# ChalmersPhotonicsLab/QAMpy

Hardware: AMD Instinct MI355X
Metric: equalised MSym/s (2-pol, 2 SPS) (higher is better)
Workload: dtype f32

## Files before the change

qampy_amd/csrc/api.hip:

```cpp
#include "common.h"
#include <stdlib.h>
#include <atomic>
#include <mutex>
#include <vector>
#include <unordered_map>
#include <string.h>

namespace qh {

thread_local hipStream_t g_stream = nullptr;
static thread_local hipStream_t g_streams[4] = {nullptr, nullptr, nullptr, nullptr};
int g_device = -1;
static thread_local std::string g_err;
static std::mutex g_mu;

void set_error(const std::string &s) { g_err = s; }

int hip_fail(hipError_t e, const char *what, const char *file, int line)
{
    g_err = std::string(hipGetErrorString(e)) + " in " + what + " (" + file + ":" + std::to_string(line) + ")";
    (void)hipGetLastError();
    return QH_ERR_HIP;
}

// ... 53 lines not shown
            const int reserved = reserved_cus();
            const int ncu = prop.multiProcessorCount;
            if (reserved > 0 && reserved < ncu) {
                std::vector<uint32_t> mask((ncu + 31) / 32, 0u);
                for (int c = reserved; c < ncu; c++) mask[c / 32] |= 1u << (c % 32);
                if (hipExtStreamCreateWithCUMask(&g_streams[i], (uint32_t)mask.size(), mask.data()) == hipSuccess) continue;
                (void)hipGetLastError();
                g_streams[i] = nullptr;
            }
        }
        QH_HIP(hipStreamCreateWithPriority(&g_streams[i], hipStreamNonBlocking, i == 2 ? prio_least : prio_greatest));
    }
    g_stream = g_streams[0];
    g_device = device;
    return QH_OK;
}

hipStream_t side_stream() { return g_stream == g_streams[0] ? g_streams[1] : g_streams[0]; }
hipStream_t helper_stream() { return g_streams[3]; }

int ensure_init()
{
    if (g_stream) return QH_OK;
    return init_device(g_device >= 0 ? g_device : 0);
}

thread_local void *g_scratch[SCRATCH_SLOTS] = {nullptr};
thread_local size_t g_scratch_n[SCRATCH_SLOTS] = {0};
thread_local unsigned g_scratch_epoch = 0;
static std::atomic<int> g_form[FORM_COUNT];
struct FormName { const char *key, *env; };
static const FormName FORM_NAMES[FORM_COUNT] = {
    {"trainer", "QAMPY_HIP_TRAINER"}, {"pit_form", "QAMPY_HIP_PIT_FORM"}, {"seg_lanes", "QAMPY_HIP_SEG_LANES"}, {"pit_probe", "QAMPY_HIP_PIT_PROBE"},
    {"bps", "QAMPY_HIP_BPS"}, {"pit_tail", "QAMPY_HIP_PIT_TAIL"}};
static int form_parse(int k, const char *v, int *out)
{
    if (!v || !v[0]) { *out = 0; return 0; }
    switch (k) {
    case FORM_TRAINER: *out = v[0] == 'd' ? 1 : (v[0] == 'l' ? 2 : (v[0] == 'i' ? 3 : (v[0] == 'a' || v[0] == '0' ? 0 : -1))); break;
    case FORM_PIT: *out = v[0] == 's' ? 1 : (v[0] == 'b' ? 2 : (v[0] == 'a' || v[0] == '0' ? 0 : -1)); break;
    case FORM_SEG_LANES: { const int n = atoi(v); *out = (n == 8 || n == 16 || n == 0) ? n : -1; break; }
    case FORM_BPS: *out = v[0] == 't' ? 1 : (v[0] == 'l' ? 2 : (v[0] == 'a' || v[0] == '0' ? 0 : -1)); break;
    case FORM_PIT_TAIL: *out = v[0] == 's' ? 1 : (v[0] == 'a' || v[0] == '0' ? 0 : -1); break;
    default: *out = atoi(v) != 0 ? 1 : 0; break;
    }
    return *out < 0 ? -1 : 0;
}
static const int g_form_env_read = [] {
    for (int k = 0; k < FORM_COUNT; k++) {
        int v = 0;
        if (form_parse(k, getenv(FORM_NAMES[k].env), &v) == 0) g_form[k].store(v);
    }
    return 0;
}();
int form(FormKey k) { return g_form[k].load(std::memory_order_relaxed); }
const char *trainer_force()
{
    switch (form(FORM_TRAINER)) {
    case 1: return "direct";
    case 2: return "lookahead";
    case 3: return "iterative";
    default: return "";
    }
}
static constexpr int POOL_CLASSES = 48, POOL_KEEP = 8;
static constexpr size_t POOL_BYTES = (size_t)24 << 30;
static std::vector<void *> g_pool[POOL_CLASSES];
static size_t g_pool_bytes = 0;
static void pool_release();
static int pool_class(size_t bytes) { int k = 8; while (((size_t)1 << k) < bytes && k < POOL_CLASSES - 1) k++; return k; }
int pool_alloc(size_t bytes, void **p, size_t *cap)
{
    const int k = pool_class(bytes);
    *cap = (size_t)1 << k;
    {
        std::lock_guard<std::mutex> lk(g_mu);
// ... 360 lines not shown
```

qampy_amd/csrc/common.h:

```cpp
#pragma once
#include <hip/hip_runtime.h>
#include <stdint.h>
#include <string>
#include "../../include/qampy_hip.h"

namespace qh {

extern thread_local hipStream_t g_stream;
extern int g_device;
void set_error(const std::string &s);
int hip_fail(hipError_t e, const char *what, const char *file, int line);

#define QH_HIP(call)                                                        \
    do {                                                                    \
        hipError_t _e = (call);                                             \
        if (_e != hipSuccess) return qh::hip_fail(_e, #call, __FILE__, __LINE__); \
    } while (0)

#define QH_REQUIRE(cond, msg)                                   \
    do {                                                        \
        if (!(cond)) { qh::set_error(msg); return QH_ERR_ARG; } \
    } while (0)

#define QH_WAVE_FIRST() __builtin_amdgcn_s_setprio(3)

int ensure_init();
hipStream_t side_stream();
hipStream_t helper_stream();
enum FormKey { FORM_TRAINER = 0, FORM_PIT, FORM_SEG_LANES, FORM_PIT_PROBE, FORM_BPS, FORM_PIT_TAIL, FORM_COUNT };
int form(FormKey k);
const char *trainer_force();
double gram_budget_gb();
int pit_timing_mode();
int default_tier();
double default_tier_tol();
constexpr int SCRATCH_SLOTS = 27;
constexpr int SCRATCH_TWOSTAGE = 16;
constexpr int SCRATCH_FOE = 17;
constexpr int SCRATCH_IMPAIR = 18;
constexpr int SCRATCH_PMD = 19;
constexpr int SCRATCH_TXRESP = 20;
constexpr int SCRATCH_SOS = 21;
constexpr int SCRATCH_CPR = 22;
constexpr int SCRATCH_FFT = 23;
constexpr int SCRATCH_SYNC = 24;
constexpr int SCRATCH_PEAK = 25;
constexpr int SCRATCH_PILOT = 26;
int scratch(int slot, size_t bytes, void **p);
unsigned scratch_epoch();

int bps_twostage_recover_f32(const void *E, int nm, int64_t L, const void *angles, int A, int B, const void *symbols, int M, int N, int32_t *idx1,
                             int32_t *idx2, void *ph, void *Eout);
int bps_twostage_recover_f64(const void *E, int nm, int64_t L, const void *angles, int A, int B, const void *symbols, int M, int N, int32_t *idx1,
                             int32_t *idx2, void *ph, void *Eout);

template <typename R> int fft_correlate_pow2(const void *x, int rows, int64_t nx, void *yrev, int64_t ny, int64_t P, void *spec, void *cc, int64_t n);

int pool_alloc(size_t bytes, void **p, size_t *cap);
void pool_free(void *p, size_t cap);

struct DevBuf {
    void *p = nullptr;
// ... 109 lines not shown
```

qampy_amd/csrc/train_pit.h:

```cpp
#pragma once
#include <atomic>
#include <chrono>
#include <vector>
#include "train_impl.h"
#include "train_seg.h"

namespace qh {

typedef qh_pit_report PitCtrl;

constexpr double PIT_CONTRACT = 0.2;
constexpr int PIT_PROBE = 128;
constexpr int PIT_SEEDWIN = 512;
constexpr int PIT_MAXSEG = 65536;

__host__ __device__ inline int pit_symmetry(int method)
{
    switch (method) {
    case QH_M_CMA: case QH_M_SGNCMA: case QH_M_RDE: return 0;
    case QH_M_CMA2: return 2;
    default: return 4;
    }
}

// ... 1973 lines not shown
            tp.wx = wx; tp.err = err; tp.mu = mu_acq; tp.nseg = 1; tp.seg_begin = step0; tp.seg_len = pl.CH; tp.seg_iter = 0; tp.skip = &ctrl->acq_done;
            rc = launch_any<R>(tp);
        }
        if (rc) return rc;
        hipLaunchKernelGGL((pit_acq_monitor_kernel<R>), dim3(1), dim3(256), 0, g_stream, (const Cx<R> *)err, err_pitch, step0, pl.CH, nsel, modes_dev,
                           pl.plateau, ctrl, mu_acq, mu_dev, pl.anneal);
    }
    return QH_OK;
}

struct PitPrepLayout { size_t ctrl, mu_acq, modes, wx, w0, err, gram, total; int64_t err_pitch; };
template <typename R> inline PitPrepLayout pit_prep_layout(int nmodes, int ntaps, int64_t acq_steps)
{
    PitPrepLayout l;
    auto up = [](size_t x) { return (x + 255) / 256 * 256; };
    const size_t wset = (size_t)nmodes * nmodes * ntaps * sizeof(Cx<R>);
    l.err_pitch = (acq_steps + LA_B + 63) / 64 * 64;
    l.ctrl = 0; l.mu_acq = up(sizeof(PitCtrl)); l.modes = l.mu_acq + 64; l.wx = up(l.modes + 128); l.w0 = up(l.wx + wset);
    l.err = up(l.w0 + wset); l.gram = up(l.err + (size_t)nmodes * l.err_pitch * sizeof(Cx<R>));
    l.total = up(l.gram + gram_bytes<R>(l.err_pitch));
    return l;
}
template <typename R> __global__ void __launch_bounds__(256) pit_adopt_kernel(Cx<R> *wx, const Cx<R> *wx_prep, int n, const PitCtrl *p, PitCtrl *c, R *mu_acq, const R *mu_acq_prep)
{
    QH_WAVE_FIRST();
    const int i = blockIdx.x * blockDim.x + threadIdx.x;
    if (!p->diverged && i < n) wx[i] = wx_prep[i];
    if (i == 0) {
        c->acq_chunks = p->acq_chunks; c->acq_steps = p->acq_steps; c->acq_done = 1; c->diverged = p->diverged; c->mu_acq = p->mu_acq;
        for (int q = 0; q < QH_PIT_MAXCHUNK; q++) c->acq_err[q] = p->acq_err[q];
        *mu_acq = *mu_acq_prep;
    }
}
template <typename R>
int pit_prepare(const void *E, int nmodes, int64_t L, int64_t TrSyms, int os, const R *mu_dev, const void *wx0, int ntaps, const int64_t *modes, int nsel,
                const void *symbols, int64_t nsy, int method, const qh_pit_opts *opts, void *prep, size_t prep_bytes)
{
    int rc = ensure_init();
    if (rc) return rc;
    if ((rc = train_args_ok("pit prepare", method, nmodes, ntaps, os, TrSyms, 1, nsel, nsy, modes))) return rc;
    QH_REQUIRE(opts && prep, "pit prepare: options and a preparation buffer are needed");
    QH_REQUIRE(TrSyms >= 1, "pit prepare: bad sizes");
    QH_REQUIRE((TrSyms - 1) * os + ntaps <= L, "pit prepare: field shorter than TrSyms*os + ntaps");
    const qh_pit_opts &o = *opts;
    QH_REQUIRE(o.acquire != 0 && o.adaptive == 0 && o.segments > 1 && o.mu_hint > 0 && o.acq_chunk > 0 && o.head_steps == 0 && !o.exchange,
               "pit prepare: not preparable (a cold fixed-step sweep with segments, mu_hint and acq_chunk given)");
    const int ntot = nmodes * ntaps;
    const PitPlan pl = pit_plan(o, TrSyms, 0, o.segments, false, o.acq_chunk);
    const PitSeg &sg = pl.sg;
    QH_REQUIRE(sg.S >= 2, "pit prepare: not preparable (nothing to parallelise)");
    const char *not_prep = "pit prepare: not preparable (throughput-form passes, block-form acquisition, blind error function)";
    QH_REQUIRE(!(method == QH_M_SBD || method == QH_M_MDDMA || method == QH_M_DD || method == QH_M_SBD_DATA), not_prep);
    TrainerForm f;
    if ((rc = trainer_form<R>(f, FORM_PASSES, method, 0, nmodes, ntaps, os, sg.len, (int64_t)sg.S * nsel, symbols, nsy, modes, nsel))) return rc;
    QH_REQUIRE(f.seg && f.block && la_shape_ok(nmodes, ntaps, os), not_prep);
    const PitPrepLayout lay = pit_prep_layout<R>(nmodes, ntaps, pl.amax);
    QH_REQUIRE(prep_bytes >= lay.total, "pit prepare: preparation buffer too small (qh_pit_prepare_bytes)");
    char *pb = (char *)prep;
    PitCtrl *ctrl = (PitCtrl *)(pb + lay.ctrl);
    R *mu_acq = (R *)(pb + lay.mu_acq);
    int64_t *modes_dev = (int64_t *)(pb + lay.modes);
    Cx<R> *wxp = (Cx<R> *)(pb + lay.wx), *w0 = (Cx<R> *)(pb + lay.w0), *errp = (Cx<R> *)(pb + lay.err);
    const size_t wset = (size_t)nmodes * ntot, wbytes = wset * sizeof(Cx<R>);
    const int64_t npow = L < 4096 ? L : 4096;
    hipLaunchKernelGGL((pit_setup_kernel<R>), dim3(1), dim3(256), 0, g_stream, (const Cx<R> *)E, nmodes, L, npow, ntot, mu_dev, pl.gear, pl.bound, o.tol > 0 ? o.tol : 1e-3, sg, ctrl, mu_acq);
    PitInit init{};
    init.cd[0] = wxp; init.cs[0] = wx0; init.cn[0] = (unsigned)wbytes;
    init.cd[1] = w0; init.cs[1] = wx0; init.cn[1] = (unsigned)wbytes;
    init.modes_dev = modes_dev; init.nsel = nsel;
    for (int j = 0; j < 16; j++) init.modes[j] = j < nsel ? modes[j] : 0;
    hipLaunchKernelGGL(pit_init_kernel, dim3(32), dim3(256), 0, g_stream, init);
    QH_REQUIRE(pl.ngram <= lay.err_pitch, "pit prepare: acquisition range exceeds the preparation buffer");
    void *G = nullptr;
    rc = f.pair_tab ? gram_build<R>(E, nmodes, L, os, ntaps, pl.ngram, &G, 1, 0, 0, pb + lay.gram) : QH_ERR_ARG;
    if (rc) return rc;
    LaArgs<R> la = la_args<R>(E, L, nmodes, ntaps, os, modes, nsel, method, symbols, nsy, mu_acq, errp, lay.err_pitch);
    la.G = (const GramPair<R> *)G; la.gpair = 1;
    if ((rc = pit_acq_enqueue<R>(pl, &la, f.use_bi, nullptr, wxp, errp, lay.err_pitch, ctrl, mu_acq, mu_dev, modes_dev, nsel))) return rc;
    hipLaunchKernelGGL((pit_acq_finish_kernel<R>), dim3((unsigned)((wset + 255) / 256)), dim3(256), 0, g_stream, wxp, (const Cx<R> *)w0, (int)wset, ctrl);
    QH_HIP(hipGetLastError());
    return QH_OK;
}

template <typename R>
int train_pit_dev(const void *E, int nmodes, int64_t L, int64_t TrSyms, int Niter, int os, R *mu_dev, void *wx, int ntaps,
                  const int64_t *modes, int nsel, const void *symbols, int64_t nsy, int method, void *err, int zero_err,
                  const void *gram, const qh_pit_opts *opts, void *report_dev, int depth = 0)
{
    pit_last_launch() = PitLaunch{0, 0, 0, 0, 0, 0};
    int rc = ensure_init();
    if (rc) return rc;
    if ((rc = train_args_ok("train_equaliser", method, nmodes, ntaps, os, TrSyms, Niter, nsel, nsy, modes))) return rc;
    QH_REQUIRE(TrSyms == 0 || (TrSyms - 1) * os + ntaps <= L, "train_equaliser: field shorter than TrSyms*os + ntaps");
    qh_pit_opts o = opts ? *opts : pit_opts_default();
    auto exact_form = [&](PitCtrl *c, int ad, int zero, const void *g, int passes) -> int {
        int r = train_dev<R>(E, nmodes, L, TrSyms, Niter, os, mu_dev, wx, ntaps, modes, nsel, ad, symbols, nsy, method, err, zero, g);
        if (r) return r;
        const int32_t hdr[3] = {1, passes, 2};
        if (passes < 0) QH_HIP(hipMemcpyAsync(&c->converged, &hdr[2], sizeof(int32_t), hipMemcpyHostToDevice, g_stream));
        else QH_HIP(hipMemcpyAsync(&c->segments, hdr, sizeof(hdr), hipMemcpyHostToDevice, g_stream));
        QH_HIP(hipStreamSynchronize(g_stream));
        return QH_OK;
    };
    QH_REQUIRE(o.segments >= 0 && o.segments <= PIT_MAXSEG && o.max_passes >= 0 && o.max_passes <= QH_PIT_MAXPASS, "train_equaliser: bad segment / pass count");
    QH_REQUIRE(o.adaptive >= 0 && o.adaptive <= 2, "train_equaliser: adaptive must be 0, 1 or 2");
    bool adaptive = o.adaptive != 0;
    {
        bool exact_only = method == QH_M_SBD_DATA;
        if (adaptive && (o.adaptive == 2 || sizeof(R) != 4 || nsel != 1 || Niter != 1 || !seg_adaptive_supported(method))) exact_only = true;
        QH_REQUIRE(!(adaptive && o.exchange), "train_equaliser: a capture split over processes is trained with a fixed step");
        if (exact_only) {
            QH_REQUIRE(!o.exchange, "train_equaliser: a capture split over processes needs the parallel-in-time solver (blind / decision-directed method, fixed step)");
            void *cb0 = nullptr;
            if ((rc = scratch(8, sizeof(PitCtrl) + 64, &cb0))) return rc;
            PitCtrl *c0 = report_dev ? (PitCtrl *)report_dev : (PitCtrl *)cb0;
            PitSeg s1; s1.S = 1; s1.len = TrSyms; s1.extra = 0; s1.tail = 0;
            hipLaunchKernelGGL((pit_setup_kernel<R>), dim3(1), dim3(256), 0, g_stream, (const Cx<R> *)E, nmodes, L, (int64_t)(L < 4096 ? L : 4096), nmodes * ntaps, (const R *)mu_dev, 1.0, 1.0,
                               o.tol > 0 ? o.tol : 1e-3, s1, c0, (R *)((char *)cb0 + sizeof(PitCtrl)));
            return exact_form(c0, o.adaptive, zero_err, adaptive ? nullptr : gram, 0);
        }
    }
    if (adaptive) o.acquire = 0;
    const int ntot = nmodes * ntaps;
    const int npass = o.max_passes > 0 ? o.max_passes : (adaptive ? QH_PIT_MAXPASS : 16);
    const double tol = (o.tol > 0 ? o.tol : 1e-3) * (adaptive ? 1.0 / 3.0 : 1.0);
    const double safety = o.dev_safety > 0 ? o.dev_safety : PIT_DEV_SAFETY;
    const int sym = pit_symmetry(method);
    const bool seed_phase = o.phase_seed < 0 ? sym == 4 : o.phase_seed != 0;
    const bool want_corr = o.correction != 0 && pit_basis_ok(ntot, sizeof(Cx<R>));
    double beta = o.corr_beta >= 0 ? o.corr_beta : (sym == 0 ? 1.5 : 0.0);

    void *cbuf = nullptr;
    if ((rc = scratch(8, sizeof(PitCtrl) + 64, &cbuf))) return rc;
    PitCtrl *ctrl = report_dev ? (PitCtrl *)report_dev : (PitCtrl *)cbuf;
    R *mu_acq = (R *)((char *)cbuf + sizeof(PitCtrl));

    int S = o.segments;
    const float ad_relax = 1.0f, ad_damp = 0.7f;
    const int ad_newton = 1;
    const int64_t head_want = 16384;
    int64_t head = adaptive ? ((TrSyms / 4 < head_want ? TrSyms / 4 : head_want) / LA_B * LA_B) : 0;
    if (!adaptive && o.head_steps > 0) {
        QH_REQUIRE(!o.exchange, "train_equaliser: a capture split over processes takes no exact head");
        head = (int64_t)o.head_steps / LA_B * LA_B;
        if (head > TrSyms) head = TrSyms / LA_B * LA_B;
        o.acquire = 0;
    }
    int64_t seg_want = 2048;
    if (adaptive && !(method == QH_M_SBD || method == QH_M_MDDMA || method == QH_M_DD)) {
        const int64_t t = ((TrSyms - head) / 512 + LA_B - 1) / LA_B * LA_B;
        if (t > seg_want) seg_want = t;
    }
    if (S == 0 && adaptive) S = (int)((TrSyms - head) / seg_want < PIT_MAXSEG ? (TrSyms - head) / seg_want : PIT_MAXSEG);
    if (S == 0) {
        R mu_h = (R)o.mu_hint;
        if (!(o.mu_hint > 0)) {
            QH_HIP(hipMemcpyAsync(&mu_h, mu_dev, sizeof(R), hipMemcpyDeviceToHost, g_stream));
            QH_HIP(hipStreamSynchronize(g_stream));
        }
        S = pit_auto_segments(TrSyms, (double)mu_h, nsel, o.acquire);
    }
    PitPlan pl = pit_plan(o, TrSyms, head, S, adaptive, o.acquire ? o.acq_chunk : 0);
    const PitSeg &sg = pl.sg;
    if (zero_err) QH_HIP(hipMemsetAsync(err, 0, (size_t)nmodes * TrSyms * Niter * sizeof(Cx<R>), g_stream));
    const int64_t npow = L < 4096 ? L : 4096;
    hipLaunchKernelGGL((pit_setup_kernel<R>), dim3(1), dim3(256), 0, g_stream, (const Cx<R> *)E, nmodes, L, npow, ntot, (const R *)mu_dev, pl.gear, pl.bound, tol, sg, ctrl, mu_acq);
    QH_HIP(hipGetLastError());
    if (TrSyms == 0 || Niter == 0) return QH_OK;
    if (sg.S < 2) {
        const double zero = 0;
        QH_HIP(hipMemcpyAsync(&ctrl->defect[0], &zero, sizeof(double), hipMemcpyHostToDevice, g_stream));
        return exact_form(ctrl, adaptive ? 1 : 0, 0, gram, 1);
    }

    TrainerForm f;
    if ((rc = trainer_form<R>(f, FORM_PASSES, method, adaptive, nmodes, ntaps, os, sg.len, (int64_t)sg.S * nsel, symbols, nsy, modes, nsel))) return rc;
    if (adaptive && !f.seg) return exact_form(ctrl, 1, 0, nullptr, 0);
    const bool decision = method == QH_M_SBD || method == QH_M_MDDMA || method == QH_M_DD;
    const bool seg_form = f.seg, use_bi = f.use_bi, block_form = f.block, pair_tab = f.pair_tab;
    const bool split = o.exchange != nullptr;
    const int own_first = split ? o.seg_first : 0, own_count = split ? o.seg_count : sg.S;
    const bool xchg_async = split && o.exchange_on_stream != 0;
    if (split) {
        QH_REQUIRE(seg_form, "train_equaliser: a capture split over processes needs the throughput form of the passes (>= 512 chains, supported tap layout)");
        QH_REQUIRE(own_first >= 0 && own_count >= 0 && own_first + own_count <= sg.S, "train_equaliser: owned segments outside the segment grid");
        QH_REQUIRE(Niter == 1, "train_equaliser: a capture split over processes is trained in one sweep");
    }

    const size_t wset = (size_t)nmodes * ntot;
    const size_t wbytes = wset * sizeof(Cx<R>);
    void *wbuf = nullptr;
    const size_t nsj = (size_t)sg.S * nsel;
    const size_t bytes_w = ((2 * (size_t)sg.S + 2) * wbytes + 63) / 64 * 64;
    if ((rc = scratch(2, bytes_w + 10 * nsj * sizeof(double) + (size_t)nsel * sizeof(int64_t) + 320 + nsj * 16 + 4 * ((nsj + 63) / 64) * sizeof(float) + 64, &wbuf))) return rc;
    Cx<R> *X = (Cx<R> *)wbuf, *Y = X + (size_t)sg.S * wset, *w_start = Y + (size_t)sg.S * wset, *w_call = w_start + wset;
    double *z = (double *)((char *)wbuf + bytes_w), *rot = z + 2 * nsj, *dfc = rot + 2 * nsj, *pw = dfc + nsj, *gph = pw + nsj, *theta = gph + 2 * nsj;
    int64_t *modes_dev = (int64_t *)(theta + 2 * nsj);
    double *uw_phi = (double *)(modes_dev + ((nsel + 7) / 8 * 8));
    int *uw_jump = (int *)(uw_phi + (size_t)sg.S * nsel);
    float *devmax = (float *)(uw_jump + (size_t)sg.S * nsel);
    const int ndev = (int)((nsj + 63) / 64);
    unsigned *ticket = (unsigned *)(devmax + 4 * (size_t)ndev);
    PitInit init{};
    init.z[0] = ticket; init.zn[0] = sizeof(unsigned);
    R *ad_rS = nullptr, *ad_rE = nullptr;
    Cx<R> *ad_eS = nullptr, *ad_eE = nullptr, *ad_errh = nullptr;
    float *ad_M = nullptr, *ad_chg = nullptr, *ad_rP = nullptr, *ad_dP = nullptr;
    if (!adaptive && head > 0) {
        void *ab = nullptr;
        if ((rc = scratch(13, (size_t)nmodes * head * sizeof(Cx<R>) + 64, &ab))) return rc;
        ad_errh = (Cx<R> *)ab;
    }
    if (adaptive) {
        void *ab = nullptr;
        const size_t nS = ((size_t)sg.S + 15) / 16 * 16;
        if ((rc = scratch(13, nS * (2 * sizeof(R) + 2 * sizeof(Cx<R>) + 3 * sizeof(float)) + 64 + (size_t)nmodes * head * sizeof(Cx<R>), &ab))) return rc;
        ad_eS = (Cx<R> *)ab; ad_eE = ad_eS + nS; ad_errh = ad_eE + nS;
        ad_rS = (R *)(ad_errh + (size_t)nmodes * head); ad_rE = ad_rS + nS;
        ad_M = (float *)(ad_rE + nS); ad_rP = ad_M + nS; ad_dP = ad_rP + nS; ad_chg = ad_dP + nS;
    }
    init.modes_dev = modes_dev; init.nsel = nsel;
    for (int j = 0; j < 16; j++) init.modes[j] = j < nsel ? modes[j] : 0;
    const bool prepared = o.prepared != nullptr && o.acquire && !adaptive && head == 0 && Niter >= 1;
    const bool need_mu = adaptive || !(o.mu_hint > 0), need_acq = o.acquire && !(o.acq_chunk > 0) && !prepared;
    R mu_acq_h = 0;
    if (need_acq) QH_HIP(hipMemcpyAsync(&mu_acq_h, mu_acq, sizeof(R), hipMemcpyDeviceToHost, g_stream));
    R mu_host = need_mu ? (R)1 : (R)o.mu_hint;
    if (need_mu) QH_HIP(hipMemcpyAsync(&mu_host, mu_dev, sizeof(R), hipMemcpyDeviceToHost, g_stream));
    if (need_mu || need_acq) QH_HIP(hipStreamSynchronize(g_stream));
    if (!adaptive && !(mu_host != 0))
        return exact_form(ctrl, 0, 0, gram, 0);
    if (o.acquire && !(o.acq_chunk > 0)) pl.acquisition(o, TrSyms, pit_acq_chunk(mu_acq_h));

    const int64_t amax = pl.amax;
    void *G = const_cast<void *>(gram);
    if (prepared) QH_REQUIRE(seg_form && o.acq_chunk > 0, "train_equaliser: a prepared acquisition belongs to throughput-form passes with acq_chunk given (qh_pit_prepare_*_dev said so)");
    if (block_form && !G && (!seg_form || amax > 0) && !prepared) {
        const int64_t n = seg_form ? pl.ngram : TrSyms;
        rc = pair_tab ? gram_build<R>(E, nmodes, L, os, ntaps, n, &G) : gram_cur_build<R>(E, nmodes, L, os, ntaps, n, &G);
        if (rc) return rc;
    }
    const int64_t g_per_step = pair_tab ? LA_B : GRAM_TRI / 2 / LA_B;

    const int ncol = sg.S * nsel;
    const double *lam = nullptr;
    const Zf *Vb = nullptr;
    Zf *Dz[2] = {nullptr, nullptr};
    Zf *Xe = nullptr, *Ye = nullptr, *Yprev = nullptr;
    if (want_corr) {
        void *cb = nullptr;
        if ((rc = scratch(10, pit_basis_bytes(ntot) + 4 * (size_t)ntot * ncol * sizeof(Zf) + (size_t)ntot * nsel * sizeof(Zf) + 256, &cb))) return rc;
        void *basis = o.basis ? o.basis : cb;
        if (!o.basis && (rc = pit_basis<R>(E, nmodes, L, os, ntaps, TrSyms, basis))) return rc;
        lam = (const double *)basis; Vb = (const Zf *)((const char *)basis + (size_t)ntot * sizeof(double));
        Dz[0] = (Zf *)((char *)cb + (pit_basis_bytes(ntot) + 63) / 64 * 64); Dz[1] = Dz[0] + (size_t)ntot * ncol;
        Xe = Dz[1] + (size_t)ntot * ncol; Ye = Xe + (size_t)ntot * ncol; Yprev = Ye + (size_t)ntot * ncol;
    }
// ... 18 lines not shown
        model = (PitModel *)((char *)uqv + b_uq); ma.model = model; ma.ticket = (unsigned *)(model + 16);
        init.z[1] = ma.ticket; init.zn[1] = sizeof(unsigned);
        init.z[2] = ualpha; init.zn[2] = (unsigned)(b_ua + b_uq);
        ma.E = (const Cx<R> *)E; ma.wx = (const Cx<R> *)wx; ma.L = L; ma.TrSyms = TrSyms; ma.nmodes = nmodes; ma.ntaps = ntaps; ma.os = os; ma.nsel = nsel; ma.method = method;
        if (decision) { ma.symbols = (const Cx<R> *)f.dd_table; ma.nsy = 2 * f.dd_npart + 1; ma.sy_pitch = 2 * BI_DD_MAXLEV; ma.tables = 1; }
        else { ma.symbols = (const Cx<R> *)symbols; ma.nsy = nsy; ma.sy_pitch = nsy; ma.tables = (method == QH_M_RDE || method == QH_M_MRDE) ? 1 : 0; }
        for (int j = 0; j < 16; j++) ma.modes[j] = j < nsel ? modes[j] : 0;
        if (o.corr_beta < 0) beta = 0.0;
    }
    const size_t glds = ((size_t)PIT_EIGMAX * PIT_EIGMAX + (size_t)PIT_EIGMAX * PIT_GT) * sizeof(Zf);
    static std::atomic<bool> gemm_attr{false};
    if (want_corr && !gemm_attr.load(std::memory_order_acquire)) {
        QH_HIP(hipFuncSetAttribute((const void *)pit_cgemm_kernel<R, true>, hipFuncAttributeMaxDynamicSharedMemorySize, 160 * 1024 - 256));
        QH_HIP(hipFuncSetAttribute((const void *)pit_cgemm_kernel<R, false>, hipFuncAttributeMaxDynamicSharedMemorySize, 160 * 1024 - 256));
        QH_HIP(hipFuncSetAttribute((const void *)pit_basis_mfma_kernel<R, 0>, hipFuncAttributeMaxDynamicSharedMemorySize, 128 * 1024));
        QH_HIP(hipFuncSetAttribute((const void *)pit_basis_mfma_kernel<R, 1>, hipFuncAttributeMaxDynamicSharedMemorySize, 128 * 1024));
        QH_HIP(hipFuncSetAttribute((const void *)pit_tail_kernel<R>, hipFuncAttributeMaxDynamicSharedMemorySize, 128 * 1024));
        gemm_attr.store(true, std::memory_order_release);
    }

    LaArgs<R> la = la_args<R>(E, L, nmodes, ntaps, os, modes, nsel, method, symbols, nsy, mu_dev, err, TrSyms * Niter);
    la.G = (const GramPair<R> *)G; la.gpair = pair_tab ? 1 : 0; la.wx_cs = (int64_t)wset;
    la.dd_general = f.dd_general;
    f.alphabet(la);
    const TrainArgs<R> ta = train_args<R>(E, L, nmodes, ntaps, os, TrSyms, Niter, modes, nsel, method, symbols, nsy, mu_dev, err);

    PitTiming &tm = pit_timing();
    tm.npass = 0; tm.acq_ms = 0;
    bool acq_timed = false;
    PitEvents &ev = pit_events();
    QH_REQUIRE(ev.ok, "train_equaliser: no pinned memory for the pass flags");
    const bool redo_ok = o.exact_redo_off == 0;
    bool fell_back = false;
    if (redo_ok && !adaptive) { init.cd[0] = w_call; init.cs[0] = wx; init.cn[0] = (unsigned)wbytes; }
    if (o.acquire && Niter > 0) { init.cd[1] = w_start; init.cs[1] = wx; init.cn[1] = (unsigned)wbytes; }
    hipLaunchKernelGGL(pit_init_kernel, dim3(32), dim3(256), 0, g_stream, init);
    QH_HIP(hipGetLastError());
    for (int it = 0; it < Niter; it++) {
        if (it == 0 && prepared) {
            const PitPrepLayout lay = pit_prep_layout<R>(nmodes, ntaps, amax);
            const char *pb = (const char *)o.prepared;
            hipLaunchKernelGGL((pit_adopt_kernel<R>), dim3((unsigned)((wset + 255) / 256)), dim3(256), 0, g_stream, (Cx<R> *)wx, (const Cx<R> *)(pb + lay.wx), (int)wset,
                               (const PitCtrl *)(pb + lay.ctrl), ctrl, mu_acq, (const R *)(pb + lay.mu_acq));
            QH_HIP(hipGetLastError());
        } else if (it == 0 && o.acquire) {
            if (pl.nchunks > 0) { QH_HIP(hipEventRecord(ev.t0[PIT_NEV - 1], g_stream)); acq_timed = true; }
            if ((rc = pit_acq_enqueue<R>(pl, block_form ? &la : nullptr, use_bi, &ta, (Cx<R> *)wx, (Cx<R> *)err, TrSyms * Niter, ctrl, mu_acq, mu_dev,
                                         modes_dev, nsel))) return rc;
            if (pl.nchunks > 0) QH_HIP(hipEventRecord(ev.t1[PIT_NEV - 1], g_stream));
            hipLaunchKernelGGL((pit_acq_finish_kernel<R>), dim3((unsigned)((wset + 255) / 256)), dim3(256), 0, g_stream, (Cx<R> *)wx, (const Cx<R> *)w_start, (int)wset, ctrl);
            QH_HIP(hipGetLastError());
        }
        if (adaptive) {
            QH_HIP(hipMemcpyAsync(w_start, wx, wbytes, hipMemcpyDeviceToDevice, g_stream));
            QH_HIP(hipMemcpyAsync(ad_chg + 1, mu_dev, sizeof(R), hipMemcpyDeviceToDevice, g_stream));
            if ((rc = train_dev<R>(E, nmodes, L, head, 1, os, mu_dev, wx, ntaps, modes, 1, 1, symbols, nsy, method, ad_errh, 0, nullptr))) return rc;
            QH_HIP(hipMemcpyAsync((Cx<R> *)err + (size_t)modes[0] * TrSyms, ad_errh + (size_t)modes[0] * head, (size_t)head * sizeof(Cx<R>), hipMemcpyDeviceToDevice, g_stream));
            hipLaunchKernelGGL((pit_adapt_init_kernel<R>), dim3((sg.S + 255) / 256), dim3(256), 0, g_stream, (const R *)mu_dev, (const Cx<R> *)(ad_errh + (size_t)modes[0] * head + head - 1),
                               sg.S, ad_rS, ad_eS);
            QH_HIP(hipGetLastError());
        }
        if (!adaptive && head > 0) {
            if ((rc = train_dev<R>(E, nmodes, L, head, 1, os, mu_dev, wx, ntaps, modes, nsel, 0, symbols, nsy, method, ad_errh, 0, nullptr))) return rc;
            for (int j = 0; j < nsel; j++)
                QH_HIP(hipMemcpyAsync((Cx<R> *)err + (size_t)modes[j] * TrSyms * Niter + (size_t)it * TrSyms, ad_errh + (size_t)modes[j] * head, (size_t)head * sizeof(Cx<R>),
                                      hipMemcpyDeviceToDevice, g_stream));
        }
        const double *rot_use = nullptr;
        if (seed_phase) {
            int nwin = PIT_SEEDWIN;
            auto phase_lds = [&](int nw) { return ((size_t)ntot + (size_t)nmodes * os * pit_phase_pitch(ntaps, os, nw)) * sizeof(Cx<R>); };
            while (nwin > 32 && phase_lds(nwin) > 60 * 1024) nwin /= 2;
            QH_REQUIRE(phase_lds(nwin) <= 60 * 1024, "train_equaliser: phase seeding does not fit the LDS for this filter shape (pass phase_seed = 0)");
            hipLaunchKernelGGL((pit_phase_kernel<R>), dim3(sg.S, nsel), dim3(256), phase_lds(nwin), g_stream, (const Cx<R> *)E, nmodes, L, os,
                               (const Cx<R> *)wx, ntaps, sg, (const int64_t *)modes_dev, nwin, z);
            hipLaunchKernelGGL(pit_unwrap_kernel, dim3(nsel), dim3(256), 0, g_stream, (const double *)z, sg.S, nsel, rot, uw_phi, uw_jump);
            rot_use = rot;
        }
        const Cx<R> *w_exact = o.start == 1 ? nullptr : ((it == 0 && o.acquire) ? (const Cx<R> *)w_start : (const Cx<R> *)wx);
        hipLaunchKernelGGL((pit_seed_kernel<R>), dim3(sg.S), dim3(256), 0, g_stream, (const Cx<R> *)wx, nmodes, ntot, (const int64_t *)modes_dev, nsel, rot_use, X, w_exact, Y, ctrl);
        if (ssb) {
            ma.sg = sg; ma.rot = rot_use;
            static thread_local hipEvent_t ev_seed = nullptr, ev_model = nullptr;
            if (!ev_seed) { QH_HIP(hipEventCreateWithFlags(&ev_seed, hipEventDisableTiming)); QH_HIP(hipEventCreateWithFlags(&ev_model, hipEventDisableTiming)); }
            hipStream_t ss = helper_stream();
            QH_HIP(hipEventRecord(ev_seed, g_stream));
            QH_HIP(hipStreamWaitEvent(ss, ev_seed, 0));
            hipLaunchKernelGGL((pit_model_kernel<R, 0>), dim3(PIT_MODB), dim3(256), 0, ss, ma);
            hipLaunchKernelGGL((pit_model_kernel<R, 1>), dim3(PIT_MODB), dim3(256), 0, ss, ma);
            QH_HIP(hipEventRecord(ev_model, ss));
            model_event = ev_model;
        }
        QH_HIP(hipGetLastError());
        const int timing_mode = pit_timing_mode();
        auto decide_args = [&](int p, const float *dm, const float2 *ye, float2 *yprev, int ne, int ncol_e, int corr_wanted) {
            PitDecideArgs<R> d;
            d.dfc = dfc; d.pw = pw; d.nb = (int)((sg.S - 1) * nsel); d.Ylast = (const Cx<R> *)(Y + (size_t)(sg.S - 1) * wset); d.n = (int)wset; d.wx = (Cx<R> *)wx; d.c = ctrl;
            d.host_view = &ev.hview[2 * p]; d.nrow = nsel; d.devmax = dm; d.ndev = ndev; d.safety = safety; d.Ye = ye; d.Yprev = yprev; d.ne = ne; d.ncol_e = ncol_e;
            d.theta = theta; d.modes_dev = (const int64_t *)modes_dev; d.ntot_w = ntot; d.S = (int)sg.S; d.sym = sym; d.corr_wanted = corr_wanted;
            d.extra = adaptive ? (const float *)ad_chg : nullptr;
            d.Dfin = (ye && !adaptive) ? (const float2 *)Dz[1] : nullptr; d.Vfin = (const float2 *)Vb; d.lam_fin = lam;
            d.stall_from = o.correction == 0 ? QH_PIT_MAXPASS : (adaptive ? 5 : 2);
            return d;
        };
        auto timed = [&](int p) { return timing_mode == 2 || (timing_mode == 1 && p == 1); };
        int back_done_for = 0;
        auto enqueue_pass = [&](int p) -> int {
            ((volatile float *)ev.hview)[2 * p] = -1.f;
            PitFuse<R> fz;
            fz.X = X; fz.Y = Y; fz.theta = theta; fz.modes_dev = (const int64_t *)modes_dev; fz.nmodes = nmodes; fz.nsel = nsel;
            fz.damp = (adaptive && p > 1) ? ad_damp : 1.f;
            fz.x_only = tail_fused ? 1 : 0;
            if (p > 0 && tail_fused && back_done_for == p) {
// ... 264 lines not shown
```

Baseline: 1237.

## Fuse PIT setup, init and phase-seed kernels into fewer launches

Merges the single-block setup kernel and the init/copy kernel into one multi-block open kernel, and lets the open work ride as extra blocks inside a new fused phase-estimation kernel. Phase unwrapping moves into the seed kernel, which computes the cumulative quarter-turn jumps per segment, so the separate unwrap launch goes away. The phase filter now processes two selected modes per block with vectorised FMA. This is meant to cut kernel launch count and serial single-block stages on the f32 path, at the cost of redundant per-block prefix scans and more code paths gated by an env switch.

```diff
diff --git a/qampy_amd/csrc/api.hip b/qampy_amd/csrc/api.hip
--- a/qampy_amd/csrc/api.hip
+++ b/qampy_amd/csrc/api.hip
@@ -109,7 +109,7 @@
 struct FormName { const char *key, *env; };
 static const FormName FORM_NAMES[FORM_COUNT] = {
     {"trainer", "QAMPY_HIP_TRAINER"}, {"pit_form", "QAMPY_HIP_PIT_FORM"}, {"seg_lanes", "QAMPY_HIP_SEG_LANES"}, {"pit_probe", "QAMPY_HIP_PIT_PROBE"},
-    {"bps", "QAMPY_HIP_BPS"}, {"pit_tail", "QAMPY_HIP_PIT_TAIL"}};
+    {"bps", "QAMPY_HIP_BPS"}, {"pit_tail", "QAMPY_HIP_PIT_TAIL"}, {"pit_open", "QAMPY_HIP_PIT_OPEN"}};
 static int form_parse(int k, const char *v, int *out)
 {
     if (!v || !v[0]) { *out = 0; return 0; }
@@ -118,7 +118,7 @@
     case FORM_PIT: *out = v[0] == 's' ? 1 : (v[0] == 'b' ? 2 : (v[0] == 'a' || v[0] == '0' ? 0 : -1)); break;
     case FORM_SEG_LANES: { const int n = atoi(v); *out = (n == 8 || n == 16 || n == 0) ? n : -1; break; }
     case FORM_BPS: *out = v[0] == 't' ? 1 : (v[0] == 'l' ? 2 : (v[0] == 'a' || v[0] == '0' ? 0 : -1)); break;
-    case FORM_PIT_TAIL: *out = v[0] == 's' ? 1 : (v[0] == 'a' || v[0] == '0' ? 0 : -1); break;
+    case FORM_PIT_TAIL: case FORM_PIT_OPEN: *out = v[0] == 's' ? 1 : (v[0] == 'a' || v[0] == '0' ? 0 : -1); break;
     default: *out = atoi(v) != 0 ? 1 : 0; break;
     }
     return *out < 0 ? -1 : 0;
diff --git a/qampy_amd/csrc/common.h b/qampy_amd/csrc/common.h
--- a/qampy_amd/csrc/common.h
+++ b/qampy_amd/csrc/common.h
@@ -27,7 +27,7 @@
 int ensure_init();
 hipStream_t side_stream();
 hipStream_t helper_stream();
-enum FormKey { FORM_TRAINER = 0, FORM_PIT, FORM_SEG_LANES, FORM_PIT_PROBE, FORM_BPS, FORM_PIT_TAIL, FORM_COUNT };
+enum FormKey { FORM_TRAINER = 0, FORM_PIT, FORM_SEG_LANES, FORM_PIT_PROBE, FORM_BPS, FORM_PIT_TAIL, FORM_PIT_OPEN, FORM_COUNT };
 int form(FormKey k);
 const char *trainer_force();
 double gram_budget_gb();
diff --git a/qampy_amd/csrc/train_pit.h b/qampy_amd/csrc/train_pit.h
--- a/qampy_amd/csrc/train_pit.h
+++ b/qampy_amd/csrc/train_pit.h
@@ -2029,6 +2029,258 @@
         *mu_acq = *mu_acq_prep;
     }
 }
+template <typename R> struct PitOpen {
+    const Cx<R> *E; int nmodes; int64_t L, npow; int ntot; const R *mu; double gear, bound, tol; PitSeg sg; PitCtrl *c; R *mu_acq;
+    PitInit init;
+    Cx<R> *wx, *copy0, *copy1; int n;
+    const Cx<R> *wx_prep; const PitCtrl *p; const R *mu_acq_prep;
+};
+template <typename R, int NM = 2> __device__ __forceinline__ void pit_open_body(const PitOpen<R> &a, int bid, int nblk, double *red)
+{
+    const int t = threadIdx.x;
+    if (bid == 0) {
+        PitCtrl *c = a.c;
+        const PitCtrl *p = a.p;
+        double m = 0, p_mu_acq = 0;
+        R p_mu = 0;
+        int64_t p_steps = 0;
+        int p_chunks = 0, p_div = 0;
+        if (t == 0) {
+            m = (double)*a.mu;
+            if (p) { p_mu_acq = p->mu_acq; p_mu = *a.mu_acq_prep; p_steps = p->acq_steps; p_chunks = p->acq_chunks; p_div = p->diverged; }
+        }
+        const double p_err = t < QH_PIT_MAXCHUNK && p ? p->acq_err[t] : -1;
+        constexpr int NU = 16;
+        double acc = 0;
+        for (int k0 = 0; k0 < a.nmodes; k0 += NM) {
+            Cx<R> v[NM][NU];
+#pragma unroll
+            for (int mm = 0; mm < NM; mm++)
+#pragma unroll
+                for (int u = 0; u < NU; u++) {
+                    const int64_t i = t + 256 * u;
+                    const bool in = k0 + mm < a.nmodes && i < a.npow;
+                    v[mm][u] = a.E[in ? (size_t)(k0 + mm) * a.L + i : 0];
+                }
+#pragma unroll
+            for (int mm = 0; mm < NM; mm++)
+#pragma unroll
+                for (int u = 0; u < NU; u++)
+                    if (k0 + mm < a.nmodes && t + 256 * u < a.npow) acc += (double)v[mm][u].re * v[mm][u].re + (double)v[mm][u].im * v[mm][u].im;
+        }
+        if (t < QH_PIT_MAXPASS) { c->result_change[t] = -1; c->deviation[t] = -1; c->deviation_rms[t] = -1; c->deviation_taps[t] = -1; c->deviation_taps_worst[t] = -1; c->defect[t] = -1; }
+        if (t < QH_PIT_MAXCHUNK) c->acq_err[t] = p_err;
+        red[t] = acc;
+        __syncthreads();
+        for (int s = 128; s > 0; s >>= 1) {
+            if (t < s) red[t] += red[t + s];
+            __syncthreads();
+        }
+        if (t == 0) {
+            const double pw = red[0] / ((double)a.nmodes * (double)a.npow);
+            double ma = a.gear * m;
+            const double cap = a.bound / ((double)a.ntot * (pw > 1e-30 ? pw : 1e-30));
+            if (ma > cap) ma = cap;
+            if (!(ma > m)) ma = m;
+            c->segments = a.sg.S; c->seg_len = a.sg.len; c->mu = m; c->power = pw; c->tol = a.tol;
+            c->passes = 0; c->converged = 0; c->done = 0; c->corr_on = 0; c->gain = 0; c->out_power = 0;
+            c->mu_acq = p ? p_mu_acq : ma; c->acq_chunks = p_chunks; c->acq_steps = p_steps; c->acq_done = p ? 1 : 0; c->diverged = p_div;
+            *a.mu_acq = p ? p_mu : (R)ma;
+        }
+        __syncthreads();
+    }
+    if (nblk > 1 && bid == 0) return;
+    const unsigned g = (nblk > 1 ? bid - 1 : 0) * 256 + t, ng = (nblk > 1 ? nblk - 1 : 1) * 256;
+#pragma unroll
+    for (int r = 0; r < 3; r++)
+        if (a.init.z[r]) for (unsigned i = g; i < a.init.zn[r] / 4; i += ng) reinterpret_cast<uint32_t *>(a.init.z[r])[i] = 0u;
+    if ((int)g < a.init.nsel) a.init.modes_dev[g] = a.init.modes[g];
+    const bool adopt = a.p && !a.p->diverged;
+    for (unsigned e = g; e < (unsigned)a.n; e += ng) {
+        const Cx<R> v = a.wx[e];
+        if (a.copy0) a.copy0[e] = v;
+        if (a.copy1) a.copy1[e] = v;
+        if (adopt) a.wx[e] = a.wx_prep[e];
+    }
+}
+template <typename R> __global__ void __launch_bounds__(256) pit_open_kernel(PitOpen<R> a)
+{
+    QH_WAVE_FIRST();
+    __shared__ double red[256];
+    pit_open_body<R>(a, (int)blockIdx.x, (int)gridDim.x, red);
+}
+constexpr int PIT_OPEN_BLOCKS = 33;
+
+struct PitModes { int m[16]; };
+typedef float pit_f2 __attribute__((ext_vector_type(2)));
+template <typename R> __device__ __forceinline__ void pit_phase_mac(R &yr, R &yi, const Cx<R> a, const Cx<R> b)
+{
+    if constexpr (sizeof(R) == 4) {
+        pit_f2 y{yr, yi};
+        y = __builtin_elementwise_fma(pit_f2{-a.im, a.im}, pit_f2{b.im, b.re}, y);
+        y = __builtin_elementwise_fma(pit_f2{a.re, a.re}, pit_f2{b.re, b.im}, y);
+        yr = y.x; yi = y.y;
+    } else {
+        yr = fma_(a.re, b.re, fma_(-a.im, b.im, yr));
+        yi = fma_(a.re, b.im, fma_(a.im, b.re, yi));
+    }
+}
+template <typename R, int NO, int NJ>
+__device__ __forceinline__ void pit_phase_filter(const Cx<R> *xs, int pitch, const Cx<R> *__restrict__ w0, const Cx<R> *__restrict__ w1, int nmodes, int os, int ntaps, const int *at,
+                                                 R (*yr)[2], R (*yi)[2])
+{
+    constexpr int CH = 4;
+    for (int k = 0; k < nmodes; k++)
+        for (int r = 0; r < os; r++) {
+            const Cx<R> *xp = xs + ((size_t)k * os + r) * pitch;
+            const Cx<R> *wr[2] = {w0 + k * ntaps + r, w1 + k * ntaps + r};
+            const int nu = (ntaps - r + os - 1) / os;
+            int u = 0;
+            for (; u + CH <= nu; u += CH) {
+                Cx<R> b[NJ][CH], a[NO][CH];
+#pragma unroll
+                for (int jj = 0; jj < NJ; jj++)
+#pragma unroll
+                    for (int c = 0; c < CH; c++) b[jj][c] = wr[jj][(u + c) * os];
+#pragma unroll
+                for (int m = 0; m < NO; m++)
+#pragma unroll
+                    for (int c = 0; c < CH; c++) a[m][c] = xp[at[m] + u + c];
+#pragma unroll
+                for (int c = 0; c < CH; c++)
+#pragma unroll
+                    for (int jj = 0; jj < NJ; jj++)
+#pragma unroll
+                        for (int m = 0; m < NO; m++) pit_phase_mac<R>(yr[jj][m], yi[jj][m], a[m][c], b[jj][c]);
+            }
+            for (; u < nu; u++) {
+#pragma unroll
+                for (int m = 0; m < NO; m++) {
+                    const Cx<R> a = xp[at[m] + u];
+#pragma unroll
+                    for (int jj = 0; jj < NJ; jj++) pit_phase_mac<R>(yr[jj][m], yi[jj][m], a, wr[jj][u * os]);
+                }
+            }
+        }
+}
+template <typename R>
+__global__ void __launch_bounds__(256) pit_phase_open_kernel(const Cx<R> *E, int nmodes, int64_t L, int os, const Cx<R> *__restrict__ wx, int ntaps, PitSeg sg, PitModes modes,
+                                                             int nsel, int nwin, double *phi, PitOpen<R> open, int nopen)
+{
+    QH_WAVE_FIRST();
+    extern __shared__ __attribute__((aligned(16))) char pit_smem[];
+    double *rr = reinterpret_cast<double *>(pit_smem), *ri = rr + 256;
+    if ((int)blockIdx.x < nopen) { pit_open_body<R, 1>(open, (int)blockIdx.x, nopen, rr); return; }
+    static_assert(PIT_SEEDWIN == 512, "pit_phase_open_kernel: one or two outputs per thread");
+    const int ntot = nmodes * ntaps;
+    const int pitch = nwin + (ntaps + os - 1) / os + 1;
+    Cx<R> *xs = reinterpret_cast<Cx<R> *>(pit_smem);
+    const int blk = (int)blockIdx.x - nopen, s = blk % sg.S, j0 = 2 * (blk / sg.S);
+    const int nj = nsel - j0 < 2 ? 1 : 2;
+    const Cx<R> *w0 = wx + (size_t)modes.m[j0] * ntot, *w1 = wx + (size_t)modes.m[j0 + nj - 1] * ntot;
+    const int64_t st = sg.start(s);
+    int64_t n = sg.steps(s);
+    if (n > nwin) n = nwin;
+    const int ns = n > 0 ? (int)(n - 1) * os + ntaps : 0;
+    for (int k = 0; k < nmodes; k++) {
+        const Cx<R> *x = E + (size_t)k * L + st * os;
+        for (int g = threadIdx.x; g < ns; g += 256) xs[((size_t)k * os + g % os) * pitch + g / os] = x[g];
+    }
+    __syncthreads();
+    R yr[2][2] = {{0, 0}, {0, 0}}, yi[2][2] = {{0, 0}, {0, 0}};
+    int at[2];
+#pragma unroll
+    for (int m = 0; m < 2; m++) at[m] = (int)threadIdx.x + 256 * m < n ? (int)threadIdx.x + 256 * m : 0;
+    if (n > 256 && nj == 2) pit_phase_filter<R, 2, 2>(xs, pitch, w0, w1, nmodes, os, ntaps, at, yr, yi);
+    else if (n > 256) pit_phase_filter<R, 2, 1>(xs, pitch, w0, w1, nmodes, os, ntaps, at, yr, yi);
+    else if (n > 0 && nj == 2) pit_phase_filter<R, 1, 2>(xs, pitch, w0, w1, nmodes, os, ntaps, at, yr, yi);
+    else if (n > 0) pit_phase_filter<R, 1, 1>(xs, pitch, w0, w1, nmodes, os, ntaps, at, yr, yi);
+#pragma unroll
+    for (int jj = 0; jj < 2; jj++) {
+        if (jj < nj) {
+            double zr = 0, zi = 0;
+#pragma unroll
+            for (int m = 0; m < 2; m++) {
+                if ((int)threadIdx.x + 256 * m < n) {
+                    const double y2r = (double)yr[jj][m] * yr[jj][m] - (double)yi[jj][m] * yi[jj][m], y2i = 2.0 * yr[jj][m] * yi[jj][m];
+                    zr += y2r * y2r - y2i * y2i;
+                    zi += 2.0 * y2r * y2i;
+                }
+            }
+            __syncthreads();
+            rr[threadIdx.x] = zr; ri[threadIdx.x] = zi;
+            __syncthreads();
+            for (int q = 128; q > 0; q >>= 1) {
+                if (threadIdx.x < q) { rr[threadIdx.x] += rr[threadIdx.x + q]; ri[threadIdx.x] += ri[threadIdx.x + q]; }
+                __syncthreads();
+            }
+            if (threadIdx.x == 0) phi[(size_t)(j0 + jj) * sg.S + s] = (rr[0] == 0 && ri[0] == 0) ? 0.0 : (double)atan2f((float)-ri[0], (float)-rr[0]) / 4;
+        }
+    }
+}
+
+template <typename R>
+__global__ void __launch_bounds__(256) pit_seed_open_kernel(const Cx<R> *wx, int nmodes, int ntot, const int64_t *modes_dev, int nsel, const double *phi, int S, double *rot, Cx<R> *X,
+                                                            const Cx<R> *w0, Cx<R> *Y, PitCtrl *c)
+{
+    QH_WAVE_FIRST();
+    __shared__ int wsum[4];
+    __shared__ double rl[16][2];
+    const int s = blockIdx.x;
+    const int n = nmodes * ntot;
+    if (s == 0 && c) {
+        if (threadIdx.x == 0) { c->done = 0; c->converged = 0; c->passes = 0; }
+        for (int q = threadIdx.x; q < QH_PIT_MAXPASS; q += 256) {
+            c->result_change[q] = -1; c->deviation[q] = -1; c->deviation_rms[q] = -1; c->deviation_taps[q] = -1; c->deviation_taps_worst[q] = -1; c->defect[q] = -1;
+        }
+    }
+    const double q = 1.5707963267948966;
+    constexpr int NB = 8;
+    for (int j = 0; j < nsel; j++) {
+        const double *ph = phi + (size_t)j * S;
+        int jumps = 0;
+        for (int base = 1; base <= s; base += 256 * NB) {
+            double a[NB], b[NB];
+#pragma unroll
+            for (int u = 0; u < NB; u++) {
+                const int sp = base + 256 * u + (int)threadIdx.x;
+                a[u] = ph[(sp <= s ? sp : s) - 1]; b[u] = ph[sp <= s ? sp : s];
+            }
+#pragma unroll
+            for (int u = 0; u < NB; u++)
+                if (base + 256 * u + (int)threadIdx.x <= s) jumps += (int)rint((a[u] - b[u]) / q);
+        }
+        for (int o = 32; o > 0; o >>= 1) jumps += __shfl_xor(jumps, o);
+        if ((threadIdx.x & 63) == 0) wsum[threadIdx.x >> 6] = jumps;
+        __syncthreads();
+        if (threadIdx.x == 0) {
+            const double p = ph[s] + q * ((wsum[0] + wsum[1] + wsum[2] + wsum[3]) & 3);
+            float sn, cs;
+            sincosf((float)p, &sn, &cs);
+            rl[j][0] = cs; rl[j][1] = -sn;
+            rot[2 * ((size_t)s * nsel + j)] = cs;
+            rot[2 * ((size_t)s * nsel + j) + 1] = -sn;
+        }
+        __syncthreads();
+    }
+    const bool exact0 = s == 0 && w0 != nullptr;
+    for (int e = threadIdx.x; e < n; e += 256) {
+        const int row = e / ntot;
+        Cx<R> v = exact0 ? w0[e] : wx[e];
+        if (!exact0) {
+            for (int j = 0; j < nsel; j++)
+                if ((int)modes_dev[j] == row) {
+                    const double c = rl[j][0], d = rl[j][1];
+                    const double vr = (double)v.re * c - (double)v.im * d, vi = (double)v.re * d + (double)v.im * c;
+                    v = Cx<R>{(R)vr, (R)vi};
+                    break;
+                }
+        }
+        X[(size_t)s * n + e] = v;
+        Y[(size_t)s * n + e] = v;
+    }
+}
+
 template <typename R>
 int pit_prepare(const void *E, int nmodes, int64_t L, int64_t TrSyms, int os, const R *mu_dev, const void *wx0, int ntaps, const int64_t *modes, int nsel,
                 const void *symbols, int64_t nsy, int method, const qh_pit_opts *opts, void *prep, size_t prep_bytes)
@@ -2060,13 +2312,19 @@
     Cx<R> *wxp = (Cx<R> *)(pb + lay.wx), *w0 = (Cx<R> *)(pb + lay.w0), *errp = (Cx<R> *)(pb + lay.err);
     const size_t wset = (size_t)nmodes * ntot, wbytes = wset * sizeof(Cx<R>);
     const int64_t npow = L < 4096 ? L : 4096;
-    hipLaunchKernelGGL((pit_setup_kernel<R>), dim3(1), dim3(256), 0, g_stream, (const Cx<R> *)E, nmodes, L, npow, ntot, mu_dev, pl.gear, pl.bound, o.tol > 0 ? o.tol : 1e-3, sg, ctrl, mu_acq);
     PitInit init{};
-    init.cd[0] = wxp; init.cs[0] = wx0; init.cn[0] = (unsigned)wbytes;
-    init.cd[1] = w0; init.cs[1] = wx0; init.cn[1] = (unsigned)wbytes;
     init.modes_dev = modes_dev; init.nsel = nsel;
     for (int j = 0; j < 16; j++) init.modes[j] = j < nsel ? modes[j] : 0;
-    hipLaunchKernelGGL(pit_init_kernel, dim3(32), dim3(256), 0, g_stream, init);
+    if (form(FORM_PIT_OPEN) == 0 && sizeof(R) == 4) {
+        PitOpen<R> op{(const Cx<R> *)E, nmodes, L, npow, ntot, mu_dev, pl.gear, pl.bound, o.tol > 0 ? o.tol : 1e-3, sg, ctrl, mu_acq, init,
+                      (Cx<R> *)const_cast<void *>(wx0), wxp, w0, (int)wset, nullptr, nullptr, nullptr};
+        hipLaunchKernelGGL((pit_open_kernel<R>), dim3(PIT_OPEN_BLOCKS), dim3(256), 0, g_stream, op);
+    } else {
+        hipLaunchKernelGGL((pit_setup_kernel<R>), dim3(1), dim3(256), 0, g_stream, (const Cx<R> *)E, nmodes, L, npow, ntot, mu_dev, pl.gear, pl.bound, o.tol > 0 ? o.tol : 1e-3, sg, ctrl, mu_acq);
+        init.cd[0] = wxp; init.cs[0] = wx0; init.cn[0] = (unsigned)wbytes;
+        init.cd[1] = w0; init.cs[1] = wx0; init.cn[1] = (unsigned)wbytes;
+        hipLaunchKernelGGL(pit_init_kernel, dim3(32), dim3(256), 0, g_stream, init);
+    }
     QH_REQUIRE(pl.ngram <= lay.err_pitch, "pit prepare: acquisition range exceeds the preparation buffer");
     void *G = nullptr;
     rc = f.pair_tab ? gram_build<R>(E, nmodes, L, os, ntaps, pl.ngram, &G, 1, 0, 0, pb + lay.gram) : QH_ERR_ARG;
@@ -2112,8 +2370,13 @@
             if ((rc = scratch(8, sizeof(PitCtrl) + 64, &cb0))) return rc;
             PitCtrl *c0 = report_dev ? (PitCtrl *)report_dev : (PitCtrl *)cb0;
             PitSeg s1; s1.S = 1; s1.len = TrSyms; s1.extra = 0; s1.tail = 0;
-            hipLaunchKernelGGL((pit_setup_kernel<R>), dim3(1), dim3(256), 0, g_stream, (const Cx<R> *)E, nmodes, L, (int64_t)(L < 4096 ? L : 4096), nmodes * ntaps, (const R *)mu_dev, 1.0, 1.0,
-                               o.tol > 0 ? o.tol : 1e-3, s1, c0, (R *)((char *)cb0 + sizeof(PitCtrl)));
+            if (form(FORM_PIT_OPEN) == 0 && sizeof(R) == 4 && !adaptive) {
+                PitOpen<R> op{(const Cx<R> *)E, nmodes, L, (int64_t)(L < 4096 ? L : 4096), nmodes * ntaps, (const R *)mu_dev, 1.0, 1.0, o.tol > 0 ? o.tol : 1e-3, s1, c0,
+                              (R *)((char *)cb0 + sizeof(PitCtrl)), PitInit{}, nullptr, nullptr, nullptr, 0, nullptr, nullptr, nullptr};
+                hipLaunchKernelGGL((pit_open_kernel<R>), dim3(1), dim3(256), 0, g_stream, op);
+            } else
+                hipLaunchKernelGGL((pit_setup_kernel<R>), dim3(1), dim3(256), 0, g_stream, (const Cx<R> *)E, nmodes, L, (int64_t)(L < 4096 ? L : 4096), nmodes * ntaps, (const R *)mu_dev, 1.0, 1.0,
+                                   o.tol > 0 ? o.tol : 1e-3, s1, c0, (R *)((char *)cb0 + sizeof(PitCtrl)));
             return exact_form(c0, o.adaptive, zero_err, adaptive ? nullptr : gram, 0);
         }
     }
@@ -2161,7 +2424,10 @@
     const PitSeg &sg = pl.sg;
     if (zero_err) QH_HIP(hipMemsetAsync(err, 0, (size_t)nmodes * TrSyms * Niter * sizeof(Cx<R>), g_stream));
     const int64_t npow = L < 4096 ? L : 4096;
-    hipLaunchKernelGGL((pit_setup_kernel<R>), dim3(1), dim3(256), 0, g_stream, (const Cx<R> *)E, nmodes, L, npow, ntot, (const R *)mu_dev, pl.gear, pl.bound, tol, sg, ctrl, mu_acq);
+    const bool prepared = o.prepared != nullptr && o.acquire && !adaptive && head == 0 && Niter >= 1;
+    const bool need_mu = adaptive || !(o.mu_hint > 0), need_acq = o.acquire && !(o.acq_chunk > 0) && !prepared;
+    const bool open_fused = form(FORM_PIT_OPEN) == 0 && sizeof(R) == 4 && !adaptive && !o.exchange && !need_mu && !need_acq && TrSyms > 0 && Niter > 0 && sg.S >= 2;
+    if (!open_fused) hipLaunchKernelGGL((pit_setup_kernel<R>), dim3(1), dim3(256), 0, g_stream, (const Cx<R> *)E, nmodes, L, npow, ntot, (const R *)mu_dev, pl.gear, pl.bound, tol, sg, ctrl, mu_acq);
     QH_HIP(hipGetLastError());
     if (TrSyms == 0 || Niter == 0) return QH_OK;
     if (sg.S < 2) {
@@ -2218,8 +2484,6 @@
     }
     init.modes_dev = modes_dev; init.nsel = nsel;
     for (int j = 0; j < 16; j++) init.modes[j] = j < nsel ? modes[j] : 0;
-    const bool prepared = o.prepared != nullptr && o.acquire && !adaptive && head == 0 && Niter >= 1;
-    const bool need_mu = adaptive || !(o.mu_hint > 0), need_acq = o.acquire && !(o.acq_chunk > 0) && !prepared;
     R mu_acq_h = 0;
     if (need_acq) QH_HIP(hipMemcpyAsync(&mu_acq_h, mu_acq, sizeof(R), hipMemcpyDeviceToHost, g_stream));
     R mu_host = need_mu ? (R)1 : (R)o.mu_hint;
@@ -2304,12 +2568,26 @@
     QH_REQUIRE(ev.ok, "train_equaliser: no pinned memory for the pass flags");
     const bool redo_ok = o.exact_redo_off == 0;
     bool fell_back = false;
-    if (redo_ok && !adaptive) { init.cd[0] = w_call; init.cs[0] = wx; init.cn[0] = (unsigned)wbytes; }
-    if (o.acquire && Niter > 0) { init.cd[1] = w_start; init.cs[1] = wx; init.cn[1] = (unsigned)wbytes; }
-    hipLaunchKernelGGL(pit_init_kernel, dim3(32), dim3(256), 0, g_stream, init);
+    PitOpen<R> open{};
+    PitModes pmodes{};
+    for (int j = 0; j < nsel; j++) pmodes.m[j] = (int)modes[j];
+    const bool open_rides = open_fused && seed_phase && !o.acquire && head == 0;
+    if (open_fused) {
+        const PitPrepLayout lay = pit_prep_layout<R>(nmodes, ntaps, amax);
+        const char *pb = (const char *)o.prepared;
+        open = PitOpen<R>{(const Cx<R> *)E, nmodes, L, npow, ntot, (const R *)mu_dev, pl.gear, pl.bound, tol, sg, ctrl, mu_acq, init, (Cx<R> *)wx,
+                          redo_ok ? w_call : nullptr, o.acquire ? w_start : nullptr, (int)wset,
+                          prepared ? (const Cx<R> *)(pb + lay.wx) : nullptr, prepared ? (const PitCtrl *)(pb + lay.ctrl) : nullptr, prepared ? (const R *)(pb + lay.mu_acq) : nullptr};
+        if (!open_rides) hipLaunchKernelGGL((pit_open_kernel<R>), dim3(PIT_OPEN_BLOCKS), dim3(256), 0, g_stream, open);
+    } else {
+        if (redo_ok && !adaptive) { init.cd[0] = w_call; init.cs[0] = wx; init.cn[0] = (unsigned)wbytes; }
+        if (o.acquire && Niter > 0) { init.cd[1] = w_start; init.cs[1] = wx; init.cn[1] = (unsigned)wbytes; }
+        hipLaunchKernelGGL(pit_init_kernel, dim3(32), dim3(256), 0, g_stream, init);
+    }
     QH_HIP(hipGetLastError());
     for (int it = 0; it < Niter; it++) {
-        if (it == 0 && prepared) {
+        if (it == 0 && prepared && open_fused) {
+        } else if (it == 0 && prepared) {
             const PitPrepLayout lay = pit_prep_layout<R>(nmodes, ntaps, amax);
             const char *pb = (const char *)o.prepared;
             hipLaunchKernelGGL((pit_adopt_kernel<R>), dim3((unsigned)((wset + 255) / 256)), dim3(256), 0, g_stream, (Cx<R> *)wx, (const Cx<R> *)(pb + lay.wx), (int)wset,
@@ -2344,13 +2622,23 @@
             auto phase_lds = [&](int nw) { return ((size_t)ntot + (size_t)nmodes * os * pit_phase_pitch(ntaps, os, nw)) * sizeof(Cx<R>); };
             while (nwin > 32 && phase_lds(nwin) > 60 * 1024) nwin /= 2;
             QH_REQUIRE(phase_lds(nwin) <= 60 * 1024, "train_equaliser: phase seeding does not fit the LDS for this filter shape (pass phase_seed = 0)");
-            hipLaunchKernelGGL((pit_phase_kernel<R>), dim3(sg.S, nsel), dim3(256), phase_lds(nwin), g_stream, (const Cx<R> *)E, nmodes, L, os,
-                               (const Cx<R> *)wx, ntaps, sg, (const int64_t *)modes_dev, nwin, z);
-            hipLaunchKernelGGL(pit_unwrap_kernel, dim3(nsel), dim3(256), 0, g_stream, (const double *)z, sg.S, nsel, rot, uw_phi, uw_jump);
+            if (open_fused) {
+                const int nopen = it == 0 && open_rides ? PIT_OPEN_BLOCKS : 0;
+                const size_t lds = std::max(phase_lds(nwin) - (size_t)ntot * sizeof(Cx<R>), (size_t)4096);
+                hipLaunchKernelGGL((pit_phase_open_kernel<R>), dim3((unsigned)(sg.S * ((nsel + 1) / 2) + nopen)), dim3(256), lds, g_stream, (const Cx<R> *)E,
+                                   nmodes, L, os, (const Cx<R> *)wx, ntaps, sg, pmodes, nsel, nwin, uw_phi, open, nopen);
+            } else {
+                hipLaunchKernelGGL((pit_phase_kernel<R>), dim3(sg.S, nsel), dim3(256), phase_lds(nwin), g_stream, (const Cx<R> *)E, nmodes, L, os,
+                                   (const Cx<R> *)wx, ntaps, sg, (const int64_t *)modes_dev, nwin, z);
+                hipLaunchKernelGGL(pit_unwrap_kernel, dim3(nsel), dim3(256), 0, g_stream, (const double *)z, sg.S, nsel, rot, uw_phi, uw_jump);
+            }
             rot_use = rot;
         }
         const Cx<R> *w_exact = o.start == 1 ? nullptr : ((it == 0 && o.acquire) ? (const Cx<R> *)w_start : (const Cx<R> *)wx);
-        hipLaunchKernelGGL((pit_seed_kernel<R>), dim3(sg.S), dim3(256), 0, g_stream, (const Cx<R> *)wx, nmodes, ntot, (const int64_t *)modes_dev, nsel, rot_use, X, w_exact, Y, ctrl);
+        if (open_fused && seed_phase)
+            hipLaunchKernelGGL((pit_seed_open_kernel<R>), dim3(sg.S), dim3(256), 0, g_stream, (const Cx<R> *)wx, nmodes, ntot, (const int64_t *)modes_dev, nsel, (const double *)uw_phi, sg.S, rot, X, w_exact, Y, ctrl);
+        else
+            hipLaunchKernelGGL((pit_seed_kernel<R>), dim3(sg.S), dim3(256), 0, g_stream, (const Cx<R> *)wx, nmodes, ntot, (const int64_t *)modes_dev, nsel, rot_use, X, w_exact, Y, ctrl);
         if (ssb) {
             ma.sg = sg; ma.rot = rot_use;
             static thread_local hipEvent_t ev_seed = nullptr, ev_model = nullptr;
```

Result: no change. 1249 (median of 4 runs) (+1.0%).
